# djeedai/bevy_hanabi

Hardware: AMD Instinct MI355X
Metric: particle-updates/sec (higher is better)
Workload: dtype f32

## Files before the change

### bevy_hanabi_amd/csrc/hanabi_amd.hip

```cpp
#include <hip/hip_runtime.h>

#include <algorithm>
#include <atomic>
#include <chrono>
#include <cmath>
#include <condition_variable>
#include <cstdarg>
#include <cstdio>
#include <cstring>
#include <deque>
#include <memory>
#include <mutex>
#include <string>
#include <thread>
#include <vector>

#include "hnb_kernels.hip.h"
#include "hnb_jit.h"
#include "hnb_sort.hip.h"
#include "hnb_comm.h"
#include "hnb_plan.h"
#include "hnb_export.h"
#include "hnb_export_code.inc"
#include "hnb_export_sort_code.inc"
// ... 220 lines not shown
    const char* stream_kernel_name = "";
    hipModule_t jit_module = nullptr;
    hipFunction_t jit_init = nullptr, jit_update = nullptr, jit_init_slots = nullptr;
    bool slot_init_eligible = false;
    uint32_t slot_init_frames = 0;
    uint32_t sort_skipped_frames = 0;
    uint32_t sort_path_frames[3] = {0, 0, 0};
    bool tick_sign_seen = false;
    uint64_t serial = 0;
    bool jit_pending = false;
    std::string kernel_info, jit_log;
    enum class StepsState { NotRequested, Built, Pending, Failed };
    hipModule_t steps_module = nullptr;
    hipFunction_t steps_update = nullptr;
    StepsState steps_state = StepsState::NotRequested;
    bool steps_from_cache = false;
    std::string steps_why;
    std::vector<Ins> steps_ops;
    int steps_waves = 0;
    bool steps_cohort = false;
    std::vector<Ins> h_init, h_update;
    std::string set_sig;
    uint64_t set_sig_hash = 0;
    uint32_t set_gen = 0, set_case = kNoSetCase, set_frames = 0;
    std::vector<Ins> uniform_code;
    std::vector<HnbEffect*> effects;
    uint32_t table_cap = 0;
    uint64_t* d_inst_base = nullptr;
    DevMeta* d_meta[2] = {nullptr, nullptr};
    struct SlabBlock { char* base = nullptr; uint32_t n_slots = 0; };
    std::vector<SlabBlock> slab_blocks;
    std::vector<void*> free_slabs;
    size_t slab_stride = 0;
    bool slot_order = false;
    bool has_ribbons = false;
    SortArgs sort{};
    uint32_t* d_plane_by_attr = nullptr;
    std::vector<uint32_t> parent_attrs;
    uint32_t* d_ev_totals = nullptr;
    unsigned long long* h_ev_counts = nullptr;
    uint32_t level = 0;
    uint32_t* d_counts = nullptr;
    uint32_t* d_deaths = nullptr;
    plan::SkipFacts skip_facts;
    plan::SkipHistory skip_hist;
    plan::RibbonFacts ribbon_facts;
    plan::RibbonHistory ribbon_hist;
    plan::FramePlan plan;
    const char* d_frame_cur = nullptr;
    uint32_t ring = 0;
    size_t frame_bytes = 0;
    uint32_t parity = 0;
    uint32_t frames_run = 0;
    uint32_t merged_frames = 0;
    uint32_t unmerged_frames = 0;
    bool horizon_eligible = false;
    uint32_t hz_parity = 0;
    uint32_t hz_frames = 0;
    uint32_t* d_safe = nullptr;
    unsigned long long* h_safe = nullptr;
    uint32_t* d_fault = nullptr;
    uint32_t skipped_frames = 0;
    uint32_t sort_parity = 0;
    uint32_t suffix_frames = 0;
    uint32_t sort_rotated_frames = 0;
    bool ring_live = false;
// ... 182 lines not shown
                break;
            case HNB_OP_M_POS_CONE3D:
                if (!OK(a, 3)) BAD("operand out of range");
                break;
            case HNB_OP_M_ADD_XLATE: break;
            case HNB_OP_LDPARENT:
                if (!is_init) BAD("LDPARENT outside the init stream");
                if (d + wd > file_regs) BAD("destination out of range");
                {
                    const uint32_t id = w[1] >> 16;
                    if (id >= HNB_ATTR_COUNT || id < HNB_ATTR_POSITION) BAD("parent attribute id out of range");
                    if (wd != kAttrComponents[id]) BAD("LDPARENT must read a whole attribute");
                    bool listed = false;
                    for (uint32_t k = 0; k < h.parent_n_attrs && !listed; ++k) {
                        uint32_t pid;
                        memcpy(&pid, blob_base + h.parent_attrs_off + k * 4, 4);
                        listed = pid == id;
                    }
                    if (!listed) BAD("LDPARENT of an attribute that is not in the program's parent attribute list");
                }
                break;
            case HNB_OP_M_EMIT_EVENTS:
                if (is_init) BAD("M_EMIT_EVENTS outside the update stream");
                if (!OK(a, 1)) BAD("operand out of range");
                if (((w[1] >> 16) & 0xffu) >= h.n_event_channels) BAD("event channel out of range");
                break;
            default: BAD("unhandled opcode");
        }
#undef BAD
    }
    return HNB_OK;
}

bool layout_slab(const HnbProgramHeader& h, const HnbAttrEntry* attrs, DevProgram& d, SortArgs& so, size_t* out_bytes) {
    d.capacity = h.capacity;
    d.n_attrs = h.n_attrs;
    d.n_uregs = h.n_uregs;
    d.chunks_per_inst = (h.capacity + kChunk - 1) / kChunk;
    d.init_len = h.init_len;
    d.update_len = h.update_len;
    uint64_t off = 0;
    const uint64_t list_bytes = align_up((size_t)h.capacity * 4, 256);
    auto place = [&](uint64_t bytes) { const uint64_t at = off; off += bytes; return at; };
    const uint64_t a0 = place(list_bytes), a1 = place(list_bytes), dd = place(list_bytes);
    uint64_t plane[kMaxAttrs];
    for (uint32_t i = 0; i < h.n_attrs; ++i) plane[i] = place(align_up((size_t)h.capacity * attrs[i].ncomp * 4, 256));
    const uint64_t flag_off = place(align_up((size_t)h.capacity, 256));
    const uint64_t lmin_off = place(align_up((size_t)d.chunks_per_inst * 16, 256));
    const uint64_t bit_bytes = align_up((size_t)d.chunks_per_inst * (kChunk / 8), 256);
    const uint64_t died_off = place(bit_bytes), rmask_off = place(bit_bytes);
    const uint64_t hz_off = place(align_up(256 + (size_t)d.chunks_per_inst * 24, 256));
    uint64_t ev_off[HNB_MAX_EVENT_CHANNELS] = {};
    for (uint32_t c = 0; c < h.n_event_channels; ++c) ev_off[c] = place(list_bytes);
    uint64_t key_off[2] = {}, val_off[2] = {}, hist_off = 0, gsum_off = 0, bits_off = 0;
    const bool ribbons = (h.flags & HNB_PROG_HAS_RIBBONS) != 0;
    const uint32_t sort_chunks = (h.capacity + kSortTile - 1) / kSortTile;
    if (ribbons) {
        for (int i = 0; i < 2; ++i) key_off[i] = place(align_up((size_t)h.capacity * 8, 256));
        for (int i = 0; i < 2; ++i) val_off[i] = place(list_bytes);
        hist_off = place(align_up((size_t)256 * sort_chunks * 4, 256));
        gsum_off = place(align_up((size_t)8 * ((sort_chunks + kSortGroup - 1) / kSortGroup) * 256 * 4, 256));
        bits_off = place(256);
    }
    if (off > ((uint64_t)0xffffffffu << 8)) return false;
    d.alive_off[0] = soff_of(a0); d.alive_off[1] = soff_of(a1); d.dead_off = soff_of(dd);
    for (uint32_t i = 0; i < h.n_attrs; ++i) {
        d.attrs[i].plane_off = soff_of(plane[i]);
        d.attrs[i].ncomp = attrs[i].ncomp;
        d.attrs[i].reg = attrs[i].reg;
        d.attrs[i].upd_flags = attrs[i].update_flags;
    }
    d.alive_flag_off = soff_of(flag_off);
    d.lmin_off = soff_of(lmin_off);
    d.died_bits_off = soff_of(died_off); d.row_mask_off = soff_of(rmask_off);
    d.horizon_off = soff_of(hz_off);
    d.n_event_channels = h.n_event_channels;
    for (uint32_t c = 0; c < h.n_event_channels; ++c) d.ev_cnt_off[c] = soff_of(ev_off[c]);
    if (ribbons) {
        so.capacity = h.capacity; so.chunks_per_inst = sort_chunks;
        so.alive_off[0] = d.alive_off[0]; so.alive_off[1] = d.alive_off[1];
        for (int i = 0; i < 2; ++i) { so.key_off[i] = soff_of(key_off[i]); so.val_off[i] = soff_of(val_off[i]); }
        so.hist_off = soff_of(hist_off); so.gsum_off = soff_of(gsum_off); so.bits_off = soff_of(bits_off);
        so.rid_plane.v = so.age_plane.v = kNoPlane;
        for (uint32_t i = 0; i < h.n_attrs; ++i) {
            if (attrs[i].attr == HNB_ATTR_RIBBON_ID) so.rid_plane = d.attrs[i].plane_off;
            if (attrs[i].attr == HNB_ATTR_AGE) so.age_plane = d.attrs[i].plane_off;
        }
    }
    *out_bytes = (size_t)off;
    return true;
}

int validate_blob(const void* blob, size_t size, HnbProgramHeader* out_hdr) {
    if (!blob || size < sizeof(HnbProgramHeader)) return fail(HNB_ERR_BAD_PROGRAM, "program blob too small");
    HnbProgramHeader h;
    memcpy(&h, blob, sizeof h);
// ... 486 lines not shown
            ctx->break_proof = value != 0u;
            return HNB_OK;
        }
        case HNB_OPT_TRANSPOSE: ctx->transpose = value != 0u; return HNB_OK;
        case HNB_OPT_SCENE_MERGE: ctx->scene_merge = value != 0u; return HNB_OK;
        case HNB_OPT_SUFFIX_PROOF: ctx->suffix_proof = value != 0u; return HNB_OK;
        case HNB_OPT_RING_LISTS: ctx->ring_lists = value != 0u; return HNB_OK;
        case HNB_OPT_SLOT_INIT:
            if (value > 2u) return fail(HNB_ERR_INVALID_ARG, "unknown slot-init mode %u", value);
            ctx->slot_init = value;
            return HNB_OK;
        case HNB_OPT_STREAM_HINTS: ctx->stream_hints = value != 0u; return HNB_OK;
        case HNB_OPT_DIRECT_UPLOAD: ctx->direct_upload = value != 0u; return HNB_OK;
        case HNB_OPT_JIT_ASYNC: ctx->jit_async = value != 0u; return HNB_OK;
        case HNB_OPT_FUSE_STEPS: ctx->fuse_steps = value != 0u; return HNB_OK;
        case HNB_OPT_SET_MODULE:
            if (value > HNB_SET_MODULE_BACKGROUND) return fail(HNB_ERR_INVALID_ARG, "unknown set-module mode %u", value);
            ctx->set_mode = value;
            ctx->set_lookup = plan::SetLookupState();
            return HNB_OK;
        case HNB_OPT_OVERLAP_UPDATES: ctx->overlap_updates = value != 0u && ctx->side_stream && ctx->ev_fork && ctx->ev_join; return HNB_OK;
        default: return fail(HNB_ERR_INVALID_ARG, "unknown option %u", option);
    }
}

int hnb_ctx_synchronize(HnbContext* ctx) {
    if (!ctx) return fail(HNB_ERR_INVALID_ARG, "ctx is NULL");
    HIP_TRY(hipStreamSynchronize(ctx->stream));
    return HNB_OK;
}

int hnb_program_validate(const void* blob, size_t blob_size) { return validate_blob(blob, blob_size, nullptr); }

int hnb_program_create(HnbContext* ctx, const void* blob, size_t blob_size, HnbProgram** out_prog) {
    if (!ctx || !out_prog) return fail(HNB_ERR_INVALID_ARG, "NULL argument");
    HnbProgramHeader h;
    int rc = validate_blob(blob, blob_size, &h);
    if (rc != HNB_OK) return rc;
    HIP_TRY(hipSetDevice(ctx->device));
    const uint8_t* b = static_cast<const uint8_t*>(blob);
    HnbProgram* p = new HnbProgram();
    p->ctx = ctx;
    p->hdr = h;
    p->attrs.resize(h.n_attrs);
    memcpy(p->attrs.data(), b + h.attrs_off, h.n_attrs * sizeof(HnbAttrEntry));
    p->props.resize(h.n_props);
    if (h.n_props) memcpy(p->props.data(), b + h.props_off, h.n_props * sizeof(HnbPropEntry));

    DevProgram& d = p->dev;
    size_t slab_bytes = 0;
    p->update_streams = update_is_streamable(b, h, p->attrs.data());
    if (!layout_slab(h, p->attrs.data(), d, p->sort, &slab_bytes)) { delete p; return fail(HNB_ERR_BAD_PROGRAM, "effect slab exceeds 1 TiB (capacity %u)", h.capacity); }
    p->slot_order = ctx->list_order == HNB_LIST_ORDER_SLOT && !(h.flags & HNB_PROG_HAS_RIBBONS);
    p->has_ribbons = (h.flags & HNB_PROG_HAS_RIBBONS) != 0;
    p->slab_bytes = slab_bytes;
    p->parent_attrs.resize(h.parent_n_attrs);
    if (h.parent_n_attrs) memcpy(p->parent_attrs.data(), b + h.parent_attrs_off, (size_t)h.parent_n_attrs * 4);
    {
        uint32_t planes[HNB_ATTR_COUNT];
        for (uint32_t i = 0; i < HNB_ATTR_COUNT; ++i) planes[i] = kNoPlane;
        for (uint32_t i = 0; i < h.n_attrs; ++i) planes[p->attrs[i].attr] = d.attrs[i].plane_off.v;
        hipError_t pe = hipMalloc(&p->d_plane_by_attr, sizeof planes);
        if (pe != hipSuccess) { delete p; return fail(HNB_ERR_OUT_OF_MEMORY, "hipMalloc failed: %s", hipGetErrorString(pe)); }
        hipMemcpy(p->d_plane_by_attr, planes, sizeof planes, hipMemcpyHostToDevice);
    }
    p->uniform_code.resize(h.uniform_len);
    if (h.uniform_len) memcpy(p->uniform_code.data(), b + h.uniform_off, (size_t)h.uniform_len * 8);
    p->wide_file = std::max(h.init_regs, h.update_regs) > HNB_VM_MAX_REGS;
    p->slot_init_eligible = slot_init_eligible(b, h);
    if (cull_eligible(b, h, p->attrs.data(), p->update_streams, ctx->popt, &p->cull_dt_operand)) {
        d.cull_lifetime = 1u;
        d.age_cohort = age_cohort_eligible(b, h, p->attrs.data(), p->update_streams, ctx->popt) ? 1u : 0u;
    }
    p->age_cohort_mode = ctx->popt.age_cohort;
    p->auto_materialise = ctx->popt.age_cohort == HNB_AGE_COHORT_AUTO && d.age_cohort != 0u && (h.render_reads_lo >> HNB_ATTR_AGE & 1u) != 0u;
    if (p->update_streams) select_stream_kernel(reinterpret_cast<const Ins*>(b + h.update_off), h.update_len, &p->stream_launch, &p->stream_kernel_name, &p->stream_launch_fused);
    if (!p->wide_file && jit::enabled()) {
        p->h_init.assign(reinterpret_cast<const Ins*>(b + h.init_off), reinterpret_cast<const Ins*>(b + h.init_off) + h.init_len);
        p->h_update.assign(reinterpret_cast<const Ins*>(b + h.update_off), reinterpret_cast<const Ins*>(b + h.update_off) + h.update_len);
        p->set_sig = jit::set_signature(make_set_request(p->h_init.data(), h.init_len, p->h_update.data(), h.update_len, p->attrs.data(), h.n_attrs, p->update_streams, d.age_cohort != 0u));
        p->set_sig_hash = jit::fnv1a(p->set_sig);
    }
    const bool aot_static = p->update_streams && strcmp(p->stream_kernel_name, "ProgInterp") != 0;
    p->kernel_info = std::string(p->wide_file ? "wide-file " : "") + "init=" + (h.init_len ? "interp" : "none") + " update=" +
                     (p->update_streams ? (aot_static ? std::string("aot-stream:") + p->stream_kernel_name : std::string("interp-stream")) : std::string("interp-generic"));
    p->serial = ctx->next_program_serial++;
    if (jit::enabled()) {
        const jit::Request rq = make_jit_request(b, h, p->attrs.data(), p->update_streams, aot_static, ctx->popt);
        if (rq.want_update_stream) {
            p->steps_ops.assign(rq.update, rq.update + rq.update_len);
            p->steps_waves = rq.stream_waves; p->steps_cohort = rq.stream_cohort;
        }
        jit::Result res;
        if (jit::build(rq, res, ctx->jit_async)) {
            install_program_jit(p, res);
        } else if (ctx->jit_async && res.log.empty() && (rq.want_init || rq.want_update_generic || rq.want_update_stream)) {
            std::unique_ptr<JitJob> job(new JitJob());
            job->program_serial = p->serial;
            job->blob.assign(b, b + blob_size);
            job->hdr = h; job->attrs = p->attrs; job->streams = p->update_streams; job->aot_static = aot_static; job->opt = ctx->popt;
            queue_jit_job(ctx, std::move(job));
            p->jit_pending = true;
        } else if (!res.log.empty()) {
            p->jit_log = res.log;
        }
    }
    if (p->has_ribbons && p->update_streams) {
// ... 81 lines not shown
        hipFree(p->d_plane_by_attr); hipFree(p->d_fault); hipHostFree(p->h_safe);
        delete p;
        return fail(HNB_ERR_OUT_OF_MEMORY, "hipMalloc(code) failed: %s", hipGetErrorString(e));
    }
    if (h.init_len) hipMemcpy(p->d_code, b + h.init_off, (size_t)h.init_len * 8, hipMemcpyHostToDevice);
    if (h.update_len) hipMemcpy(p->d_code + h.init_len, b + h.update_off, (size_t)h.update_len * 8, hipMemcpyHostToDevice);
    d.init_code = p->d_code;
    d.update_code = p->d_code + h.init_len;
    ctx->programs.push_back(p);
    *out_prog = p;
    return HNB_OK;
}

int hnb_program_destroy(HnbProgram* p) {
    if (!p) return HNB_OK;
    HnbContext* ctx = p->ctx;
    hipSetDevice(ctx->device);
    hipStreamSynchronize(ctx->stream);
    while (!p->effects.empty()) hnb_effect_destroy(p->effects.back());
    free_tables(p);
    if (p->jit_module) hipModuleUnload(p->jit_module);
    if (p->steps_module) hipModuleUnload(p->steps_module);
    for (auto& blk : p->slab_blocks) hipFree(blk.base);
    hipFree(p->d_plane_by_attr);
    hipFree(p->d_code);
    hipFree(p->d_fault);
    hipFree(p->d_export);
    if (p->h_safe) hipHostFree(p->h_safe);
    ctx->programs.erase(std::remove(ctx->programs.begin(), ctx->programs.end(), p), ctx->programs.end());
    delete p;
    return HNB_OK;
}

constexpr size_t kPlacementMinBytes = (size_t)256 << 20;
constexpr size_t kPlacementMaxTransient = (size_t)32 << 30;
hipError_t alloc_slab_block(HnbProgram* p, size_t bytes, char** out) {
    int want = 24;
    if (const char* e = getenv("HNB_SLAB_CANDIDATES")) want = std::max(1, std::min(32, atoi(e)));
    want = (int)std::min<size_t>((size_t)want, std::max<size_t>(1, kPlacementMaxTransient / std::max<size_t>(bytes, 1)));
    if (bytes < kPlacementMinBytes || bytes != p->slab_stride) want = 1;
    const bool debug = getenv("HNB_DEBUG_ALLOC") != nullptr;
    if (want == 1) return hipMalloc(reinterpret_cast<void**>(out), bytes);
    ProbeArgs pa{};
    pa.n_quads = (p->dev.capacity + 3u) / 4u;
    for (uint32_t a = 0; a < p->dev.n_attrs && pa.n_planes < 8; ++a) {
        const DevAttr& at = p->dev.attrs[a];
        if (at.reg == HNB_REG_NONE) continue;
        pa.off[pa.n_planes] = at.plane_off;
        pa.stride16[pa.n_planes] = at.ncomp;
        if (at.reg != HNB_REG_LIFETIME) pa.write_mask |= 1u << pa.n_planes;
        pa.n_planes += 1;
    }
    hipStream_t st = p->ctx->stream;
    hipEvent_t ev0 = nullptr, ev1 = nullptr;
    if (hipEventCreate(&ev0) != hipSuccess || hipEventCreate(&ev1) != hipSuccess) {
        if (ev0) hipEventDestroy(ev0);
        (void)hipGetLastError();
        return hipMalloc(reinterpret_cast<void**>(out), bytes);
    }
    char* best = nullptr;
    float best_ms = 0.0f;
    std::vector<float> times;
    std::vector<char*> rejected;
    hipError_t first_error = hipSuccess;
    for (int c = 0; c < want; ++c) {
        char* cand = nullptr;
        const hipError_t e = hipMalloc(reinterpret_cast<void**>(&cand), bytes);
        if (e != hipSuccess) { if (!best) first_error = e; (void)hipGetLastError(); break; }
        hipMemsetAsync(cand, 0, bytes, st);
        float ms = 1e30f;
        const uint32_t grid = (uint32_t)((pa.n_quads + 255u) / 256u);
        for (int rep = 0; rep < 4; ++rep) {
            hipEventRecord(ev0, st);
            k_probe_placement<<<grid, 256, 0, st>>>(cand, pa);
            hipEventRecord(ev1, st);
            hipEventSynchronize(ev1);
            float t = 0.0f;
            hipEventElapsedTime(&t, ev0, ev1);
            if (rep > 0 && t < ms) ms = t;
        }
        if (debug) fprintf(stderr, "hanabi_amd: slab candidate %d at %p: %.4f ms\n", c, (void*)cand, ms);
        if (!best || ms < best_ms) { if (best) rejected.push_back(best); best = cand; best_ms = ms; }
        else rejected.push_back(cand);
        times.push_back(ms);
        if (times.size() >= 3) {
            std::vector<float> sorted = times;
            std::sort(sorted.begin(), sorted.end());
            if (best_ms < 0.97f * sorted[sorted.size() / 2]) break;
        }
    }
    for (char* r : rejected) hipFree(r);
    hipEventDestroy(ev0);
    hipEventDestroy(ev1);
    if (!best) return first_error;
    *out = best;
    return hipSuccess;
}

int hnb_effect_create(HnbProgram* p, uint32_t slot_base, HnbEffect** out_fx) {
    if (!p || !out_fx) return fail(HNB_ERR_INVALID_ARG, "NULL argument");
    HnbContext* ctx = p->ctx;
    HIP_TRY(hipSetDevice(ctx->device));
    const uint32_t index = (uint32_t)p->effects.size();
    int rc = ensure_tables(p, index + 1);
    if (rc != HNB_OK) return rc;
    HIP_TRY(hipStreamSynchronize(ctx->stream));
    HnbEffect* fx = new HnbEffect();
    fx->prog = p;
    fx->index = index;
    fx->slot_base = slot_base;
    hipError_t e = hipSuccess;
    if (p->free_slabs.empty()) {
        p->slab_stride = align_up(p->slab_bytes, 64 * 1024);
        const size_t want = std::max<size_t>(1, ((size_t)1 << 30) / p->slab_stride);
        const uint32_t n_slots = (uint32_t)std::min<size_t>(want, std::max<size_t>(1, p->effects.size()));
        HnbProgram::SlabBlock blk;
        blk.n_slots = n_slots;
        e = alloc_slab_block(p, p->slab_stride * n_slots, &blk.base);
        if (e == hipSuccess) {
            p->slab_blocks.push_back(blk);
            for (uint32_t i = n_slots; i-- > 0;) p->free_slabs.push_back(blk.base + (size_t)i * p->slab_stride);
        }
    }
    if (e == hipSuccess) { fx->slab = p->free_slabs.back(); p->free_slabs.pop_back(); }
    if (e == hipSuccess && getenv("HNB_DEBUG_ALLOC")) fprintf(stderr, "hanabi_amd: effect slab %p (%zu bytes)\n", fx->slab, p->slab_bytes);
    if (e != hipSuccess) { delete fx; return fail(HNB_ERR_OUT_OF_MEMORY, "hipMalloc(%zu bytes) for effect slab failed: %s", p->slab_bytes, hipGetErrorString(e)); }
    char* base = static_cast<char*>(fx->slab);
    const uint32_t cap = p->dev.capacity;
// ... 1601 lines not shown
    if (!fx) return fail(HNB_ERR_INVALID_ARG, "fx is NULL");
    if (!fx->prog->has_ribbons) return fail(HNB_ERR_INVALID_ARG, "the particle layout has no RIBBON_ID attribute: nothing to sort");
    return HNB_OK;
}

int hnb_program_kernel_info(HnbProgram* prog, char* buf, size_t buf_size) {
    if (!prog || !buf || !buf_size) return fail(HNB_ERR_INVALID_ARG, "NULL argument");
    std::string s = prog->kernel_info;
    if (prog->jit_pending) s += " (specialisation pending: HNB_OPT_JIT_ASYNC)";
    if (!prog->jit_log.empty()) s += "\njit log: " + prog->jit_log;
    {
        const char* never = steps_never_reason(prog);
        s += "\nsteps kernel: ";
        switch (prog->steps_state) {
        case HnbProgram::StepsState::NotRequested: s += std::string("not requested") + (never ? std::string(" (") + never + ")" : std::string()); break;
        case HnbProgram::StepsState::Built: s += std::string("built") + (prog->steps_from_cache ? " (jit cache hit)" : ""); break;
        case HnbProgram::StepsState::Pending: s += "pending (HNB_OPT_JIT_ASYNC)"; break;
        case HnbProgram::StepsState::Failed: s += "failed: " + prog->steps_why; break;
        }
    }
    if (!prog->dev.age_cohort && prog->dev.cull_lifetime && prog->age_cohort_mode == HNB_AGE_COHORT_AUTO && (prog->hdr.render_reads_lo >> HNB_ATTR_AGE & 1u))
        s += "\nage cohorts: off (HNB_AGE_COHORT_AUTO: the asset's render modifiers read AGE after every frame)";
    if (prog->dev.age_cohort) {
        hipStreamSynchronize(prog->ctx->stream);
        std::vector<uint32_t> st(prog->dev.chunks_per_inst);
        size_t in_cohort = 0;
        for (const HnbEffect* fx : prog->effects) {
            if (hipMemcpy(st.data(), static_cast<const char*>(fx->slab) + prog->dev.lmin_off + (size_t)prog->dev.chunks_per_inst * 8, st.size() * 4, hipMemcpyDeviceToHost) != hipSuccess) break;
            for (uint32_t v : st) in_cohort += v == 1u ? 1u : 0u;
        }
        s += "\nage cohorts: " + std::to_string(in_cohort) + " of " + std::to_string(prog->effects.size() * (size_t)prog->dev.chunks_per_inst) + " chunks";
        if (prog->auto_materialise) s += " (HNB_AGE_COHORT_AUTO: the asset's render modifiers read AGE, the update keeps the plane current)";
    }
    if (prog->slot_init_frames) s += "\nslot-major init (large spawns): " + std::to_string(prog->slot_init_frames) + " frames";
    if (prog->has_ribbons && prog->suffix_frames) s += "\ncasualties proven to be the list's last rows (no k_count_rows): " + std::to_string(prog->suffix_frames) + " frames";
    if (prog->has_ribbons && prog->ring_frames) s += "\nlist kept as a ring (no row rewritten): " + std::to_string(prog->ring_frames) + " frames";
    if (prog->has_ribbons && prog->sort_skipped_frames) s += "\nribbon sorts skipped in list-free frames: " + std::to_string(prog->sort_skipped_frames) + " frames";
    if (prog->has_ribbons) s += "\nribbon sorts by rotation: " + std::to_string(prog->sort_rotated_frames) + " of " + std::to_string(prog->frames_run) + " frames" + (prog->ribbon_facts.front_static ? "" : " (not eligible)");
    if (prog->has_ribbons) s += "\nribbon sorts by path: one-tile " + std::to_string(prog->sort_path_frames[0]) + ", one-workgroup " + std::to_string(prog->sort_path_frames[1]) +
                                ", multi-launch " + std::to_string(prog->sort_path_frames[2]) + " frames";
    if (prog->merged_frames) s += "\nupdate served by a merged launch (small programs of the context share one): " + std::to_string(prog->merged_frames) + " frames";
    if (prog->unmerged_frames) s += "\nkept out of the shared launches (the loaded set module does not know this program; its own specialised kernels): " + std::to_string(prog->unmerged_frames) + " frames";
    if (prog->set_frames) s += "\n... by the context's set module (the program's specialised code behind the shared launch): " + std::to_string(prog->set_frames) + " frames";
    if (!prog->ctx->set_log.empty() && !prog->set_sig.empty()) s += "\nset module: " + prog->ctx->set_log;
    if (prog->ctx->set_failed_builds && !prog->set_sig.empty()) s += "\nset module builds that failed: " + std::to_string(prog->ctx->set_failed_builds);
    if (prog->horizon_eligible) s += "\ndeath horizons in use: " + std::to_string(prog->hz_frames) + " frames";
    s += "\nlists skipped: " + std::to_string(prog->skipped_frames) + " of " + std::to_string(prog->frames_run) + " frames" + (prog->skip_facts.eligible ? "" : " (not eligible)");
    s += "\nframe parameters (context): written by the host into device memory in " + std::to_string(prog->ctx->direct_frames) + " frames, copied in " + std::to_string(prog->ctx->copied_frames) +
         (prog->ctx->large_bar ? "" : " (the device memory is not host-visible: no large BAR)") + (prog->ctx->direct_failed ? " (host-visible slots failed their check)" : "");
    s += "\nhnb_simulate waited for the device (the frame " + std::to_string(kFrameRing) + " before still running) in " + std::to_string(prog->ctx->ring_waits) + " of " + std::to_string(prog->ctx->frame) +
         " frames, " + std::to_string(prog->ctx->ring_wait_ns / 1000) + " us in all";
    snprintf(buf, buf_size, "%s", s.c_str());
    return HNB_OK;
}

int hnb_jit_precompile(const void* blob, size_t blob_size) {
    HnbProgramHeader h;
    int rc = validate_blob(blob, blob_size, &h);
    if (rc != HNB_OK) return rc;
    const uint8_t* b = static_cast<const uint8_t*>(blob);
    std::vector<HnbAttrEntry> attrs(h.n_attrs);
    memcpy(attrs.data(), b + h.attrs_off, h.n_attrs * sizeof(HnbAttrEntry));
    const bool streams = update_is_streamable(b, h, attrs.data());
    bool aot_static = false;
    if (streams) {
        StreamLaunchFn fn = nullptr;
// ... 271 lines not shown
```

### bevy_hanabi_amd/csrc/hnb_kernels.hip.h

```cpp
#pragma once
#ifndef __HIPCC_RTC__
#include <hip/hip_runtime.h>
#endif
#include "hnb_dev.h"

namespace hnb {

template <class T>
__device__ __forceinline__ T* global_ptr(uint64_t addr) {
    typedef __attribute__((address_space(1))) T global_t;
    return (T*)(global_t*)addr;
}

struct u2_t { uint32_t x, y; };
struct u3_t { uint32_t x, y, z; };
typedef uint32_t u4v __attribute__((ext_vector_type(4)));
#if defined(HNB_NONTEMPORAL) || defined(HNB_NONTEMPORAL_LOADS)
#define HNB_NT_LOAD(p) __builtin_nontemporal_load(p)
#else
#define HNB_NT_LOAD(p) (*(p))
#endif
#if defined(HNB_NONTEMPORAL) || defined(HNB_NONTEMPORAL_STORES)
#define HNB_NT_STORE(v, p) __builtin_nontemporal_store(v, p)
#else
// ... 15 lines not shown
    HNB_WAVE_STEP_(v, ident, OP, 0x142, 0xa)                \
    HNB_WAVE_STEP_(v, ident, OP, 0x143, 0xc)
__device__ __forceinline__ uint32_t wave_sum_u32(uint32_t v) {
#define HNB_OP_(a, b) ((a) + (b))
    HNB_WAVE_REDUCE_(v, 0u, HNB_OP_)
#undef HNB_OP_
    return (uint32_t)__builtin_amdgcn_readlane((int)v, 63);
}
__device__ __forceinline__ uint32_t wave_min_u32(uint32_t v) {
#define HNB_OP_(a, b) ((b) < (a) ? (b) : (a))
    HNB_WAVE_REDUCE_(v, 0xffffffffu, HNB_OP_)
#undef HNB_OP_
    return (uint32_t)__builtin_amdgcn_readlane((int)v, 63);
}
__device__ __forceinline__ uint32_t wave_max_u32(uint32_t v) {
#define HNB_OP_(a, b) ((b) > (a) ? (b) : (a))
    HNB_WAVE_REDUCE_(v, 0u, HNB_OP_)
#undef HNB_OP_
    return (uint32_t)__builtin_amdgcn_readlane((int)v, 63);
}
__device__ __forceinline__ float wave_min_f32(float x) {
    uint32_t v = f2u(x);
#define HNB_OP_(a, b) f2u(fminf(u2f(a), u2f(b)))
    HNB_WAVE_REDUCE_(v, 0x7f800000u, HNB_OP_)
#undef HNB_OP_
    return u2f((uint32_t)__builtin_amdgcn_readlane((int)v, 63));
}


#ifndef HNB_JIT_TU
__global__ void k_reset_lists(uint32_t* __restrict__ dead, uint32_t* __restrict__ alive0, uint32_t* __restrict__ alive1, uint32_t capacity) {
    uint32_t i = blockIdx.x * blockDim.x + threadIdx.x;
    if (i < capacity) { dead[i] = i; alive0[i] = 0u; alive1[i] = 0u; }
}
#endif

#ifndef HNB_JIT_TU
struct ProbeArgs { uint32_t n_planes; uint32_t stride16[8]; uint64_t off[8]; uint32_t write_mask; uint32_t salt; uint64_t n_quads; };
__global__ void __launch_bounds__(256) k_probe_placement(char* __restrict__ base, const ProbeArgs a) {
    const uint64_t q = (uint64_t)blockIdx.x * 256u + threadIdx.x;
    if (q >= a.n_quads) return;
    uint32_t acc = 0;
#pragma unroll
    for (uint32_t pl = 0; pl < 8; ++pl) {
        if (pl >= a.n_planes) break;
        uint4* ptr = reinterpret_cast<uint4*>(base + a.off[pl]) + q * a.stride16[pl];
        for (uint32_t i = 0; i < a.stride16[pl]; ++i) {
            uint4 v = ptr[i];
            acc += v.x + v.y + v.z + v.w;
            v.x ^= a.salt;
            if (a.write_mask >> pl & 1u) ptr[i] = v;
        }
    }
    if (acc == 0x9e3779b9u && a.salt) *reinterpret_cast<uint32_t*>(base) = acc;
}
#endif

template <class FILE_T>
__device__ __forceinline__ void vfile_store_attr(const FILE_T& r, uint32_t ncomp, uint32_t reg, char* plane, uint32_t slot) {
    switch (ncomp) {
        case 1: reinterpret_cast<uint32_t*>(plane)[slot] = r[reg]; break;
        case 2: reinterpret_cast<u2_t*>(plane)[slot] = u2_t{r[reg], r[reg + 1]}; break;
        case 3: reinterpret_cast<u3_t*>(plane)[slot] = u3_t{r[reg], r[reg + 1], r[reg + 2]}; break;
        default: reinterpret_cast<uint4*>(plane)[slot] = make_uint4(r[reg], r[reg + 1], r[reg + 2], r[reg + 3]); break;
    }
}
__device__ __forceinline__ Out4 vfile_load_attr(uint32_t ncomp, const char* plane, uint32_t slot) {
    Out4 o = Out4{0u, 0u, 0u, 0u};
    switch (ncomp) {
        case 1: o.v0 = reinterpret_cast<const uint32_t*>(plane)[slot]; break;
        case 2: { const u2_t t = reinterpret_cast<const u2_t*>(plane)[slot]; o.v0 = t.x; o.v1 = t.y; } break;
        case 3: { const u3_t t = reinterpret_cast<const u3_t*>(plane)[slot]; o.v0 = t.x; o.v1 = t.y; o.v2 = t.z; } break;
        default: { const uint4 t = reinterpret_cast<const uint4*>(plane)[slot]; o.v0 = t.x; o.v1 = t.y; o.v2 = t.z; o.v3 = t.w; } break;
    }
    return o;
}

__device__ __forceinline__ void pin_scalar(uint32_t v) { asm volatile("" ::"s"(v)); }
__device__ __forceinline__ uint32_t requested_spawn(const DevFrameInst& f) {
    const uint4 h0 = reinterpret_cast<const uint4*>(&f)[0], h1 = reinterpret_cast<const uint4*>(&f)[1];
    const uint32_t spawn_count = h0.x, parity = h1.z, skip = h1.w;
    const uint64_t ev_in = (uint64_t)h1.x | ((uint64_t)h1.y << 32);
    pin_scalar(spawn_count);
    if (skip) return 0u;
    if (ev_in == 0ull) return spawn_count;
    const DevEventBuffer* ev = global_ptr<const DevEventBuffer>(ev_in);
    const uint2 cnt = *reinterpret_cast<const uint2*>(ev->count);
// ... 1284 lines not shown
            if (next != ast_raw) astate[j] = next;
        }
        uint32_t d = 0;
#pragma unroll
        for (uint32_t w = 0; w < kBlock / 64; ++w) d += s_died[w];
        if (d) atomicAdd(&cb.deaths[(size_t)cb.parity * cb.table_cap + k], d);
        if (d && args.skip_lists) *args.fault = 1u;
        if (args.safe_words) {
            float r = fminf(fminf(s_rem[0], s_rem[1]), fminf(s_rem[2], s_rem[3]));
            r = r > 0.0f ? r : 0.0f;
            uint32_t* word = args.safe_words + (size_t)args.safe_parity * args.safe_stride + chunk;
            if (split) atomicMin(word, f2u(r));
            else *word = f2u(r);
        }
        if (chunk_full) { if (d) cfull[j] = 0u; }
        else if (!split && d == 0u && s_alive[0] + s_alive[1] + s_alive[2] + s_alive[3] == kChunk) cfull[j] = 1u;
        if (cull && !split) {
            float m = __builtin_inff();
            bool all = true;
#pragma unroll
            for (uint32_t w = 0; w < kBlock / 64; ++w) { all = all && !(s_lmin[w] < 0.0f); m = fminf(m, s_lmin[w]); }
            if (all) lmin[j] = m < 3.0e38f ? m : 3.0e38f;
        }
    }
}

template <class PROG, int WAVES, int PROBE = 0, bool COHORT = false, bool FUSED = false>
__global__ void __launch_bounds__(kBlock, WAVES)
k_update_slots_stream(const SlotArgs args, const uint64_t* __restrict__ inst_base, const DevFrameInst* __restrict__ fi,
                      const uint32_t* __restrict__ ublocks, const CompactBufs cb) {
    update_stream_chunk<PROG, PROBE, COHORT, FUSED>(args, inst_base, fi, ublocks, cb, blockIdx.x, gridDim.x);
}
#ifndef HNB_JIT_TU
#ifndef HNB_AGEK_CUT
#define HNB_AGEK_CUT 0
#endif
__global__ void __launch_bounds__(kBlock)
k_update_slots_stream_age(const SlotArgs args, const uint64_t* __restrict__ inst_base, const DevFrameInst* __restrict__ fi,
                          const uint32_t* __restrict__ ublocks, const CompactBufs cb) {
    __shared__ uint32_t s_died[kBlock / 64], s_alive[kBlock / 64];
    __shared__ float s_lmin[kBlock / 64], s_rem[kBlock / 64];
    constexpr uint32_t kSteps = kWaveRows / kStepRows;
    const uint32_t tid = threadIdx.x, lane = tid & 63u, wave = tid >> 6;
    const uint32_t wg = blockIdx.x, wg_total = gridDim.x;
    const uint32_t chunk = chunk_of_workgroup(cb.xcd_remap, wg, wg_total);
    const uint32_t k = chunk / args.chunks_per_inst, j = chunk - k * args.chunks_per_inst;
    const uint32_t frozen = fi[k].skip;
    char* base = global_ptr<char>(inst_base[k]);
    const float dt_tick = u2f(ublocks[(size_t)k * args.n_uregs + (args.dt_operand & 0xffu)]);
    char* p_age = base + args.plane_off[2];
    const char* p_life = base + args.plane_off[3];
    uint32_t* flags4 = reinterpret_cast<uint32_t*>(base + args.alive_flag_off);
    float* lmin = reinterpret_cast<float*>(base + args.lmin_off);
    uint32_t* cfull = reinterpret_cast<uint32_t*>(lmin) + args.chunks_per_inst;
    const uint32_t wave0 = j * kChunk + wave * kWaveRows;
    uint32_t f4s[kSteps];
    u4v ages[kSteps];
#pragma unroll
    for (uint32_t step = 0; step < kSteps; ++step) {
        const uint32_t s0 = wave0 + step * kStepRows + lane * 4u;
        const bool in = s0 < args.capacity;
        f4s[step] = in ? ld_hint(flags4 + (s0 >> 2), args.stream_hint != 0u) : 0u;
        ages[step] = in ? reinterpret_cast<const u4v*>(p_age)[s0 >> 2] : u4v{0u, 0u, 0u, 0u};
    }
    const uint32_t cf = cfull[j];
    const float Lm = lmin[j];
// ... 420 lines not shown
```

### bevy_hanabi_amd/csrc/hnb_plan.h

```cpp
#pragma once
#include <cstdint>
#include <cstring>

namespace hnb {
namespace plan {

struct InstanceFrame {
    bool simulated = true;
    bool has_parent = false;
    uint32_t spawn_count = 0;
    uint32_t event_capacity = 0;
    const uint32_t* ublock = nullptr;
};
inline uint32_t uword(const InstanceFrame& f, uint32_t decoded_operand) { return f.ublock[decoded_operand & 0xffu]; }
inline float as_float(uint32_t bits) { float f; std::memcpy(&f, &bits, 4); return f; }
inline bool nonneg_not_nan(uint32_t float_bits) { return float_bits <= 0x7f800000u; }

struct SkipFacts {
    bool eligible = false;
    uint32_t dt_operand = 0;
};
struct SkipHistory {
    double cum_tick[128] = {};
    uint32_t last_dirty = 0;
// ... 225 lines not shown

inline void partition_init_passes(const uint8_t* reads, uint32_t n, int heavy, uint8_t* side) {
    for (uint32_t i = 0; i < n; ++i) side[i] = heavy >= 0 ? 1u : 0u;
    if (heavy < 0) return;
    side[heavy] = 0u;
    for (uint32_t c = 0; c < n; ++c)
        if (reads[c * n + (uint32_t)heavy]) side[c] = 0u;
    for (bool changed = true; changed;) {
        changed = false;
        for (uint32_t c = 0; c < n; ++c)
            if (!side[c])
                for (uint32_t p = 0; p < n; ++p)
                    if (side[p] && reads[c * n + p]) { side[p] = 0u; changed = true; }
    }
}

struct SetLookupState { uint64_t seen = 0, tried = 0; };
inline bool set_lookup_due(SetLookupState& st, bool enabled, bool job_running, bool covered, uint32_t n_candidates, uint64_t population) {
    if (!enabled || job_running || covered || n_candidates < 2u) return false;
    if (population == st.tried) return false;
    if (population != st.seen) { st.seen = population; return false; }
    st.tried = population;
    return true;
}

constexpr uint64_t kStreamHintBytes = 256ull << 20;
inline bool use_streaming_hints(uint64_t total_slots, uint32_t update_bytes_per_slot) {
    return total_slots * (uint64_t)(update_bytes_per_slot + 8u) > kStreamHintBytes;
}

constexpr uint64_t kStoreHintBytes = 384ull << 20;
inline bool use_store_hints(uint64_t total_slots, uint32_t stored_bytes_per_slot) { return total_slots * (uint64_t)stored_bytes_per_slot > kStoreHintBytes; }

struct FramePlan {
    bool skip_lists = false;
    bool lists = true;
    bool lists_merged = false;
    bool hz_use = false;
    bool stream_hint = false;
    bool store_hint = false;
    RibbonDecision ribbon;
    bool independent = false;
    MergeDecision merge;
    uint32_t init_blocks = 0;
    SlotInitDecision slot_init;
};

}
}
```

Measured before the change: 123.1 billion.

## Make slab placement probe mimic the streaming update kernel and refine candidate selection

Reworks the physical-placement search for large effect slabs. The probe kernel now mirrors the streaming update's chunk/wave access pattern, XCD remap, occupancy and per-plane load/store masks, so candidate timings better reflect the real update. The stop rule now distinguishes a single timing class from multiple classes and keeps searching for a while after the best candidate. It also adds optional per-plane skew padding (off by default), a per-program stream-wave choice, and diagnostics. The cost is more allocation-time probing, and the probe may still mispredict real performance.

```diff
diff --git a/bevy_hanabi_amd/csrc/hanabi_amd.hip b/bevy_hanabi_amd/csrc/hanabi_amd.hip
--- a/bevy_hanabi_amd/csrc/hanabi_amd.hip
+++ b/bevy_hanabi_amd/csrc/hanabi_amd.hip
@@ -276,6 +276,10 @@
     std::vector<SlabBlock> slab_blocks;
     std::vector<void*> free_slabs;
     size_t slab_stride = 0;
+    uint32_t plane_pad[kMaxAttrs] = {};
+    int stream_waves = HNB_STREAM_WAVES;
+    uint32_t placement_tried = 0;
+    float placement_best_ms = 0.0f, placement_median_ms = 0.0f;
     bool slot_order = false;
     bool has_ribbons = false;
     SortArgs sort{};
@@ -524,36 +528,27 @@
     return HNB_OK;
 }
 
-bool layout_slab(const HnbProgramHeader& h, const HnbAttrEntry* attrs, DevProgram& d, SortArgs& so, size_t* out_bytes) {
+bool layout_slab(const HnbProgramHeader& h, const HnbAttrEntry* attrs, DevProgram& d, SortArgs& so, size_t* out_bytes, const uint32_t* pad256 = nullptr) {
     d.capacity = h.capacity;
     d.n_attrs = h.n_attrs;
     d.n_uregs = h.n_uregs;
     d.chunks_per_inst = (h.capacity + kChunk - 1) / kChunk;
     d.init_len = h.init_len;
     d.update_len = h.update_len;
-    uint64_t off = 0;
-    const uint64_t list_bytes = align_up((size_t)h.capacity * 4, 256);
-    auto place = [&](uint64_t bytes) { const uint64_t at = off; off += bytes; return at; };
-    const uint64_t a0 = place(list_bytes), a1 = place(list_bytes), dd = place(list_bytes);
-    uint64_t plane[kMaxAttrs];
-    for (uint32_t i = 0; i < h.n_attrs; ++i) plane[i] = place(align_up((size_t)h.capacity * attrs[i].ncomp * 4, 256));
-    const uint64_t flag_off = place(align_up((size_t)h.capacity, 256));
-    const uint64_t lmin_off = place(align_up((size_t)d.chunks_per_inst * 16, 256));
-    const uint64_t bit_bytes = align_up((size_t)d.chunks_per_inst * (kChunk / 8), 256);
-    const uint64_t died_off = place(bit_bytes), rmask_off = place(bit_bytes);
-    const uint64_t hz_off = place(align_up(256 + (size_t)d.chunks_per_inst * 24, 256));
-    uint64_t ev_off[HNB_MAX_EVENT_CHANNELS] = {};
-    for (uint32_t c = 0; c < h.n_event_channels; ++c) ev_off[c] = place(list_bytes);
-    uint64_t key_off[2] = {}, val_off[2] = {}, hist_off = 0, gsum_off = 0, bits_off = 0;
-    const bool ribbons = (h.flags & HNB_PROG_HAS_RIBBONS) != 0;
+    static_assert(plan::kLayoutMaxAttrs == kMaxAttrs && plan::kLayoutMaxChannels == HNB_MAX_EVENT_CHANNELS, "plan::SlabShape limits");
+    plan::SlabShape shape;
+    shape.capacity = h.capacity; shape.n_attrs = h.n_attrs; shape.n_event_channels = h.n_event_channels;
+    shape.ribbons = (h.flags & HNB_PROG_HAS_RIBBONS) != 0;
+    shape.chunk = kChunk; shape.sort_tile = kSortTile; shape.sort_group = kSortGroup;
+    for (uint32_t i = 0; i < h.n_attrs; ++i) { shape.ncomp[i] = attrs[i].ncomp; shape.pad256[i] = pad256 ? pad256[i] : 0u; }
+    const plan::SlabSections sec = plan::layout_sections(shape);
+    const uint64_t off = sec.total, a0 = sec.alive[0], a1 = sec.alive[1], dd = sec.dead;
+    const uint64_t* plane = sec.plane;
+    const uint64_t flag_off = sec.flag, lmin_off = sec.lmin, died_off = sec.died, rmask_off = sec.rmask, hz_off = sec.horizon;
+    const uint64_t* ev_off = sec.ev;
+    const uint64_t *key_off = sec.key, *val_off = sec.val, hist_off = sec.hist, gsum_off = sec.gsum, bits_off = sec.bits;
+    const bool ribbons = shape.ribbons;
     const uint32_t sort_chunks = (h.capacity + kSortTile - 1) / kSortTile;
-    if (ribbons) {
-        for (int i = 0; i < 2; ++i) key_off[i] = place(align_up((size_t)h.capacity * 8, 256));
-        for (int i = 0; i < 2; ++i) val_off[i] = place(list_bytes);
-        hist_off = place(align_up((size_t)256 * sort_chunks * 4, 256));
-        gsum_off = place(align_up((size_t)8 * ((sort_chunks + kSortGroup - 1) / kSortGroup) * 256 * 4, 256));
-        bits_off = place(256);
-    }
     if (off > ((uint64_t)0xffffffffu << 8)) return false;
     d.alive_off[0] = soff_of(a0); d.alive_off[1] = soff_of(a1); d.dead_off = soff_of(dd);
     for (uint32_t i = 0; i < h.n_attrs; ++i) {
@@ -1106,6 +1101,13 @@
 
 int hnb_program_validate(const void* blob, size_t blob_size) { return validate_blob(blob, blob_size, nullptr); }
 
+constexpr size_t kPlacementMinBytes = (size_t)256 << 20;
+constexpr uint32_t kPlaneSkewBytes = 0;
+uint32_t plane_skew_for(size_t slab_bytes) {
+    if (const char* e = getenv("HNB_PLANE_SKEW")) return (uint32_t)(std::min<long long>(std::max(0ll, atoll(e)), 1ll << 30) / 256);
+    return slab_bytes >= kPlacementMinBytes ? kPlaneSkewBytes / 256u : 0u;
+}
+
 int hnb_program_create(HnbContext* ctx, const void* blob, size_t blob_size, HnbProgram** out_prog) {
     if (!ctx || !out_prog) return fail(HNB_ERR_INVALID_ARG, "NULL argument");
     HnbProgramHeader h;
@@ -1125,6 +1127,10 @@
     size_t slab_bytes = 0;
     p->update_streams = update_is_streamable(b, h, p->attrs.data());
     if (!layout_slab(h, p->attrs.data(), d, p->sort, &slab_bytes)) { delete p; return fail(HNB_ERR_BAD_PROGRAM, "effect slab exceeds 1 TiB (capacity %u)", h.capacity); }
+    if (const uint32_t skew256 = plane_skew_for(slab_bytes)) {
+        for (uint32_t i = 1; i < h.n_attrs; ++i) p->plane_pad[i] = skew256;
+        if (!layout_slab(h, p->attrs.data(), d, p->sort, &slab_bytes, p->plane_pad)) { delete p; return fail(HNB_ERR_BAD_PROGRAM, "effect slab exceeds 1 TiB (capacity %u)", h.capacity); }
+    }
     p->slot_order = ctx->list_order == HNB_LIST_ORDER_SLOT && !(h.flags & HNB_PROG_HAS_RIBBONS);
     p->has_ribbons = (h.flags & HNB_PROG_HAS_RIBBONS) != 0;
     p->slab_bytes = slab_bytes;
@@ -1147,6 +1153,12 @@
         d.age_cohort = age_cohort_eligible(b, h, p->attrs.data(), p->update_streams, ctx->popt) ? 1u : 0u;
     }
     p->age_cohort_mode = ctx->popt.age_cohort;
+    {
+        bool lean = true;
+        for (uint32_t i = 0; i < h.update_len; ++i) lean = lean && vm_op_is_lean(reinterpret_cast<const Ins*>(b + h.update_off)[i].x & 0xffu);
+        p->stream_waves = lean ? HNB_STREAM_WAVES : HNB_STREAM_WAVES_FULL;
+        if (d.age_cohort && p->stream_waves > HNB_STREAM_WAVES_COHORT) p->stream_waves = HNB_STREAM_WAVES_COHORT;
+    }
     p->auto_materialise = ctx->popt.age_cohort == HNB_AGE_COHORT_AUTO && d.age_cohort != 0u && (h.render_reads_lo >> HNB_ATTR_AGE & 1u) != 0u;
     if (p->update_streams) select_stream_kernel(reinterpret_cast<const Ins*>(b + h.update_off), h.update_len, &p->stream_launch, &p->stream_kernel_name, &p->stream_launch_fused);
     if (!p->wide_file && jit::enabled()) {
@@ -1294,25 +1306,54 @@
     return HNB_OK;
 }
 
-constexpr size_t kPlacementMinBytes = (size_t)256 << 20;
 constexpr size_t kPlacementMaxTransient = (size_t)32 << 30;
+constexpr int kPlacementCandidates = 24;
+size_t placement_min_bytes() {
+    if (const char* e = getenv("HNB_SLAB_MIN_BYTES")) return (size_t)std::max(0ll, atoll(e));
+    return kPlacementMinBytes;
+}
+ProbeArgs probe_args_of(const HnbProgram* p) {
+    ProbeArgs pa{};
+    pa.stream = p->update_streams ? 1u : 0u;
+    pa.n_quads = ((uint64_t)p->dev.capacity + 3u) / 4u;
+    for (uint32_t a = 0; a < p->dev.n_attrs && pa.n_planes < 4; ++a) {
+        const DevAttr& at = p->dev.attrs[a];
+        if (at.reg == HNB_REG_NONE || at.ncomp > 3u) continue;
+        bool load = (at.upd_flags & HNB_ATTR_UPD_LOAD) != 0, store = (at.upd_flags & HNB_ATTR_UPD_STORE) != 0;
+        if (pa.stream) {
+            if (at.reg == HNB_REG_LIFETIME && p->dev.cull_lifetime) load = false;
+            if (at.reg == HNB_REG_AGE && p->dev.age_cohort) { load = false; store = store && p->auto_materialise; }
+        } else {
+            load = true; store = store || at.reg != HNB_REG_LIFETIME;
+        }
+        if (!load && !store) continue;
+        const uint32_t i = pa.n_planes++;
+        pa.off[i] = at.plane_off;
+        pa.ncomp[i] = at.ncomp;
+        pa.words[i] = align_up((size_t)p->dev.capacity * at.ncomp * 4, 256) / 16;
+        if (load) pa.load_mask |= 1u << i;
+        if (store) pa.store_mask |= 1u << i;
+    }
+    return pa;
+}
+void launch_probe(int waves, uint32_t grid, hipStream_t st, char* block, const ProbeArgs& pa) {
+    const size_t lds = pa.stream ? sizeof(StreamLds) : 0;
+    switch (waves) {
+    case 4: k_probe_placement<4><<<grid, kBlock, lds, st>>>(block, pa); break;
+    case 5: k_probe_placement<5><<<grid, kBlock, lds, st>>>(block, pa); break;
+    default: k_probe_placement<6><<<grid, kBlock, lds, st>>>(block, pa); break;
+    }
+}
 hipError_t alloc_slab_block(HnbProgram* p, size_t bytes, char** out) {
-    int want = 24;
+    int want = kPlacementCandidates;
     if (const char* e = getenv("HNB_SLAB_CANDIDATES")) want = std::max(1, std::min(32, atoi(e)));
     want = (int)std::min<size_t>((size_t)want, std::max<size_t>(1, kPlacementMaxTransient / std::max<size_t>(bytes, 1)));
-    if (bytes < kPlacementMinBytes || bytes != p->slab_stride) want = 1;
+    if (bytes < placement_min_bytes() || bytes != p->slab_stride) want = 1;
     const bool debug = getenv("HNB_DEBUG_ALLOC") != nullptr;
     if (want == 1) return hipMalloc(reinterpret_cast<void**>(out), bytes);
-    ProbeArgs pa{};
-    pa.n_quads = (p->dev.capacity + 3u) / 4u;
-    for (uint32_t a = 0; a < p->dev.n_attrs && pa.n_planes < 8; ++a) {
-        const DevAttr& at = p->dev.attrs[a];
-        if (at.reg == HNB_REG_NONE) continue;
-        pa.off[pa.n_planes] = at.plane_off;
-        pa.stride16[pa.n_planes] = at.ncomp;
-        if (at.reg != HNB_REG_LIFETIME) pa.write_mask |= 1u << pa.n_planes;
-        pa.n_planes += 1;
-    }
+    ProbeArgs pa = probe_args_of(p);
+    if (pa.n_planes == 0u) return hipMalloc(reinterpret_cast<void**>(out), bytes);
+    const uint32_t grid = pa.stream ? p->dev.chunks_per_inst : (uint32_t)((pa.n_quads + kBlock - 1u) / kBlock);
     hipStream_t st = p->ctx->stream;
     hipEvent_t ev0 = nullptr, ev1 = nullptr;
     if (hipEventCreate(&ev0) != hipSuccess || hipEventCreate(&ev1) != hipSuccess) {
@@ -1320,42 +1361,41 @@
         (void)hipGetLastError();
         return hipMalloc(reinterpret_cast<void**>(out), bytes);
     }
-    char* best = nullptr;
-    float best_ms = 0.0f;
     std::vector<float> times;
-    std::vector<char*> rejected;
+    std::vector<char*> cands;
     hipError_t first_error = hipSuccess;
+    plan::PlacementPick pick;
     for (int c = 0; c < want; ++c) {
         char* cand = nullptr;
         const hipError_t e = hipMalloc(reinterpret_cast<void**>(&cand), bytes);
-        if (e != hipSuccess) { if (!best) first_error = e; (void)hipGetLastError(); break; }
+        if (e != hipSuccess) { if (cands.empty()) first_error = e; (void)hipGetLastError(); break; }
         hipMemsetAsync(cand, 0, bytes, st);
         float ms = 1e30f;
-        const uint32_t grid = (uint32_t)((pa.n_quads + 255u) / 256u);
-        for (int rep = 0; rep < 4; ++rep) {
+        for (int rep = 0; rep < 5; ++rep) {
+            pa.mode = (p->ctx->alternate && (rep & 1)) ? 2u : 0u;
             hipEventRecord(ev0, st);
-            k_probe_placement<<<grid, 256, 0, st>>>(cand, pa);
+            launch_probe(p->stream_waves, grid, st, cand, pa);
             hipEventRecord(ev1, st);
-            hipEventSynchronize(ev1);
             float t = 0.0f;
-            hipEventElapsedTime(&t, ev0, ev1);
+            if (hipEventSynchronize(ev1) != hipSuccess || hipEventElapsedTime(&t, ev0, ev1) != hipSuccess) { (void)hipGetLastError(); continue; }
             if (rep > 0 && t < ms) ms = t;
         }
         if (debug) fprintf(stderr, "hanabi_amd: slab candidate %d at %p: %.4f ms\n", c, (void*)cand, ms);
-        if (!best || ms < best_ms) { if (best) rejected.push_back(best); best = cand; best_ms = ms; }
-        else rejected.push_back(cand);
+        cands.push_back(cand);
         times.push_back(ms);
-        if (times.size() >= 3) {
-            std::vector<float> sorted = times;
-            std::sort(sorted.begin(), sorted.end());
-            if (best_ms < 0.97f * sorted[sorted.size() / 2]) break;
-        }
-    }
-    for (char* r : rejected) hipFree(r);
+        pick = plan::placement_pick(times.data(), (uint32_t)times.size(), (uint32_t)want);
+        if (pick.stop) break;
+    }
     hipEventDestroy(ev0);
     hipEventDestroy(ev1);
-    if (!best) return first_error;
-    *out = best;
+    if (cands.empty()) return first_error;
+    pick = plan::placement_pick(times.data(), (uint32_t)times.size(), (uint32_t)times.size());
+    for (size_t i = 0; i < cands.size(); ++i) if (i != pick.pick) hipFree(cands[i]);
+    std::vector<float> sorted = times;
+    std::sort(sorted.begin(), sorted.end());
+    p->placement_tried = (uint32_t)times.size(); p->placement_best_ms = times[pick.pick]; p->placement_median_ms = sorted[sorted.size() / 2];
+    if (debug) fprintf(stderr, "hanabi_amd: slab placement: %u candidates, kept %u (%.4f ms, median %.4f ms)\n", p->placement_tried, pick.pick, p->placement_best_ms, p->placement_median_ms);
+    *out = cands[pick.pick];
     return hipSuccess;
 }
 
@@ -3023,6 +3063,15 @@
         s += "\nage cohorts: " + std::to_string(in_cohort) + " of " + std::to_string(prog->effects.size() * (size_t)prog->dev.chunks_per_inst) + " chunks";
         if (prog->auto_materialise) s += " (HNB_AGE_COHORT_AUTO: the asset's render modifiers read AGE, the update keeps the plane current)";
     }
+    {
+        char line[256];
+        if (prog->placement_tried) snprintf(line, sizeof line, "\nslab placement: %u candidates tried, best %.4f ms, median %.4f ms", prog->placement_tried, prog->placement_best_ms, prog->placement_median_ms);
+        else snprintf(line, sizeof line, "\nslab placement: not searched");
+        s += line;
+        s += "; plane skews (bytes):";
+        uint64_t cum = 0;
+        for (uint32_t i = 0; i < prog->dev.n_attrs; ++i) { cum += (uint64_t)prog->plane_pad[i] * 256u; s += " " + std::to_string(cum); }
+    }
     if (prog->slot_init_frames) s += "\nslot-major init (large spawns): " + std::to_string(prog->slot_init_frames) + " frames";
     if (prog->has_ribbons && prog->suffix_frames) s += "\ncasualties proven to be the list's last rows (no k_count_rows): " + std::to_string(prog->suffix_frames) + " frames";
     if (prog->has_ribbons && prog->ring_frames) s += "\nlist kept as a ring (no row rewritten): " + std::to_string(prog->ring_frames) + " frames";
diff --git a/bevy_hanabi_amd/csrc/hnb_kernels.hip.h b/bevy_hanabi_amd/csrc/hnb_kernels.hip.h
--- a/bevy_hanabi_amd/csrc/hnb_kernels.hip.h
+++ b/bevy_hanabi_amd/csrc/hnb_kernels.hip.h
@@ -71,27 +71,6 @@
 __global__ void k_reset_lists(uint32_t* __restrict__ dead, uint32_t* __restrict__ alive0, uint32_t* __restrict__ alive1, uint32_t capacity) {
     uint32_t i = blockIdx.x * blockDim.x + threadIdx.x;
     if (i < capacity) { dead[i] = i; alive0[i] = 0u; alive1[i] = 0u; }
-}
-#endif
-
-#ifndef HNB_JIT_TU
-struct ProbeArgs { uint32_t n_planes; uint32_t stride16[8]; uint64_t off[8]; uint32_t write_mask; uint32_t salt; uint64_t n_quads; };
-__global__ void __launch_bounds__(256) k_probe_placement(char* __restrict__ base, const ProbeArgs a) {
-    const uint64_t q = (uint64_t)blockIdx.x * 256u + threadIdx.x;
-    if (q >= a.n_quads) return;
-    uint32_t acc = 0;
-#pragma unroll
-    for (uint32_t pl = 0; pl < 8; ++pl) {
-        if (pl >= a.n_planes) break;
-        uint4* ptr = reinterpret_cast<uint4*>(base + a.off[pl]) + q * a.stride16[pl];
-        for (uint32_t i = 0; i < a.stride16[pl]; ++i) {
-            uint4 v = ptr[i];
-            acc += v.x + v.y + v.z + v.w;
-            v.x ^= a.salt;
-            if (a.write_mask >> pl & 1u) ptr[i] = v;
-        }
-    }
-    if (acc == 0x9e3779b9u && a.salt) *reinterpret_cast<uint32_t*>(base) = acc;
 }
 #endif
 
@@ -1442,6 +1421,81 @@
     update_stream_chunk<PROG, PROBE, COHORT, FUSED>(args, inst_base, fi, ublocks, cb, blockIdx.x, gridDim.x);
 }
 #ifndef HNB_JIT_TU
+struct ProbeArgs {
+    uint32_t n_planes;
+    uint32_t ncomp[4];
+    uint64_t off[4];
+    uint64_t words[4];
+    uint32_t load_mask, store_mask;
+    uint32_t salt;
+    uint32_t stream;
+    uint32_t mode;
+    uint64_t n_quads;
+};
+template <int WAVES>
+__global__ void __launch_bounds__(kBlock) __attribute__((amdgpu_waves_per_eu(WAVES, WAVES))) k_probe_placement(char* __restrict__ base, const ProbeArgs a) {
+    uint32_t acc = 0;
+    if (!a.stream) {
+        const uint64_t q = (uint64_t)blockIdx.x * kBlock + threadIdx.x;
+        if (q >= a.n_quads) return;
+#pragma unroll
+        for (uint32_t pl = 0; pl < 4; ++pl) {
+            if (pl >= a.n_planes || !((a.load_mask | a.store_mask) >> pl & 1u)) continue;
+            u4v* ptr = reinterpret_cast<u4v*>(base + a.off[pl]);
+            for (uint32_t i = 0; i < a.ncomp[pl]; ++i) {
+                const uint64_t g = q * a.ncomp[pl] + i;
+                if (g >= a.words[pl]) break;
+                u4v v = u4v{0u, 0u, 0u, 0u};
+                if (a.load_mask >> pl & 1u) { v = ptr[g]; acc += v.x + v.y + v.z + v.w; v.x ^= a.salt; }
+                if (a.store_mask >> pl & 1u) ptr[g] = v;
+            }
+        }
+    } else {
+        const uint32_t lane = threadIdx.x & 63u, wave = threadIdx.x >> 6;
+        const uint32_t chunk = chunk_of_workgroup(a.mode, blockIdx.x, gridDim.x);
+        constexpr uint32_t kSteps = kWaveRows / kStepRows;
+        auto word_of = [&](uint32_t pl, uint32_t step, uint32_t w) {
+            return ((uint64_t)chunk * (kChunk / 4u) + wave * (kWaveRows / 4u)) * a.ncomp[pl] + (step * a.ncomp[pl] + w) * 64u + lane;
+        };
+#pragma unroll
+        for (uint32_t pl = 0; pl < 4; ++pl) {
+            if (pl >= a.n_planes || !(a.store_mask >> pl & 1u) || (a.load_mask >> pl & 1u)) continue;
+            u4v* ptr = reinterpret_cast<u4v*>(base + a.off[pl]);
+            for (uint32_t step = 0; step < kSteps; ++step)
+                for (uint32_t w = 0; w < a.ncomp[pl]; ++w) { const uint64_t g = word_of(pl, step, w); if (g < a.words[pl]) ptr[g] = u4v{a.salt, 0u, 0u, 0u}; }
+        }
+        constexpr int kInFlight = WAVES <= 4 ? 2 : 1;
+#pragma unroll kInFlight
+        for (uint32_t step = 0; step < kSteps; ++step) {
+            u4v v[4][3];
+#pragma unroll
+            for (uint32_t pl = 0; pl < 4; ++pl) {
+                if (pl >= a.n_planes || !(a.load_mask >> pl & 1u)) continue;
+                const u4v* ptr = reinterpret_cast<const u4v*>(base + a.off[pl]);
+#pragma unroll
+                for (uint32_t w = 0; w < 3; ++w) {
+                    v[pl][w] = u4v{0u, 0u, 0u, 0u};
+                    if (w < a.ncomp[pl]) { const uint64_t g = word_of(pl, step, w); if (g < a.words[pl]) v[pl][w] = ptr[g]; }
+                }
+            }
+#pragma unroll
+            for (uint32_t pl = 0; pl < 4; ++pl) {
+                if (pl >= a.n_planes || !(a.load_mask >> pl & 1u)) continue;
+                u4v* ptr = reinterpret_cast<u4v*>(base + a.off[pl]);
+#pragma unroll
+                for (uint32_t w = 0; w < 3; ++w) {
+                    if (w >= a.ncomp[pl]) continue;
+                    acc += v[pl][w].x + v[pl][w].y + v[pl][w].z + v[pl][w].w;
+                    v[pl][w].x ^= a.salt;
+                    const uint64_t g = word_of(pl, step, w);
+                    if ((a.store_mask >> pl & 1u) && g < a.words[pl]) ptr[g] = v[pl][w];
+                }
+            }
+        }
+    }
+    if (acc == 0x9e3779b9u && a.salt) *reinterpret_cast<uint32_t*>(base + a.off[0]) = acc;
+}
+
 #ifndef HNB_AGEK_CUT
 #define HNB_AGEK_CUT 0
 #endif
diff --git a/bevy_hanabi_amd/csrc/hnb_plan.h b/bevy_hanabi_amd/csrc/hnb_plan.h
--- a/bevy_hanabi_amd/csrc/hnb_plan.h
+++ b/bevy_hanabi_amd/csrc/hnb_plan.h
@@ -281,6 +281,72 @@
 constexpr uint64_t kStoreHintBytes = 384ull << 20;
 inline bool use_store_hints(uint64_t total_slots, uint32_t stored_bytes_per_slot) { return total_slots * (uint64_t)stored_bytes_per_slot > kStoreHintBytes; }
 
+constexpr uint32_t kLayoutMaxAttrs = 40, kLayoutMaxChannels = 8;
+struct SlabShape {
+    uint32_t capacity = 0, n_attrs = 0;
+    uint32_t ncomp[kLayoutMaxAttrs] = {};
+    uint32_t pad256[kLayoutMaxAttrs] = {};
+    uint32_t n_event_channels = 0;
+    bool ribbons = false;
+    uint32_t chunk = 4096, sort_tile = 4096, sort_group = 32;
+};
+struct SlabSections {
+    uint64_t alive[2] = {}, dead = 0, plane[kLayoutMaxAttrs] = {}, flag = 0, lmin = 0, died = 0, rmask = 0, horizon = 0, ev[kLayoutMaxChannels] = {};
+    uint64_t key[2] = {}, val[2] = {}, hist = 0, gsum = 0, bits = 0;
+    uint64_t total = 0;
+};
+inline uint64_t up256(uint64_t v) { return (v + 255u) & ~(uint64_t)255u; }
+inline SlabSections layout_sections(const SlabShape& s) {
+    SlabSections o;
+    uint64_t off = 0;
+    auto place = [&](uint64_t bytes) { const uint64_t at = off; off += bytes; return at; };
+    const uint64_t list_bytes = up256((uint64_t)s.capacity * 4u);
+    const uint64_t chunks = ((uint64_t)s.capacity + s.chunk - 1u) / s.chunk;
+    o.alive[0] = place(list_bytes); o.alive[1] = place(list_bytes); o.dead = place(list_bytes);
+    for (uint32_t i = 0; i < s.n_attrs && i < kLayoutMaxAttrs; ++i) { off += (uint64_t)s.pad256[i] * 256u; o.plane[i] = place(up256((uint64_t)s.capacity * s.ncomp[i] * 4u)); }
+    o.flag = place(up256(s.capacity));
+    o.lmin = place(up256(chunks * 16u));
+    const uint64_t bit_bytes = up256(chunks * (s.chunk / 8u));
+    o.died = place(bit_bytes); o.rmask = place(bit_bytes);
+    o.horizon = place(up256(256u + chunks * 24u));
+    for (uint32_t c = 0; c < s.n_event_channels && c < kLayoutMaxChannels; ++c) o.ev[c] = place(list_bytes);
+    if (s.ribbons) {
+        const uint64_t sort_chunks = ((uint64_t)s.capacity + s.sort_tile - 1u) / s.sort_tile;
+        for (int i = 0; i < 2; ++i) o.key[i] = place(up256((uint64_t)s.capacity * 8u));
+        for (int i = 0; i < 2; ++i) o.val[i] = place(list_bytes);
+        o.hist = place(up256(256u * sort_chunks * 4u));
+        o.gsum = place(up256(8u * ((sort_chunks + s.sort_group - 1u) / s.sort_group) * 256u * 4u));
+        o.bits = place(256u);
+    }
+    o.total = off;
+    return o;
+}
+
+constexpr float kPlacementSeparation = 0.97f;
+constexpr uint32_t kPlacementStand = 12, kPlacementOneClass = 8;
+constexpr float kPlacementFailed = 1e29f;
+struct PlacementPick { bool stop = true; uint32_t pick = 0; };
+inline PlacementPick placement_pick(const float* ms, uint32_t n, uint32_t budget) {
+    PlacementPick r;
+    if (n == 0u) { r.stop = budget == 0u; return r; }
+    bool have = false;
+    float best = 0.0f, worst = 0.0f;
+    uint32_t finite = 0;
+    for (uint32_t i = 0; i < n; ++i) {
+        if (!(ms[i] < kPlacementFailed)) continue;
+        finite += 1u;
+        if (!have || ms[i] < best) { best = ms[i]; r.pick = i; }
+        if (!have || ms[i] > worst) worst = ms[i];
+        have = true;
+    }
+    if (n >= budget) { r.stop = true; return r; }
+    if (!have) { r.stop = false; return r; }
+    const bool classes = best < kPlacementSeparation * worst;
+    if (!classes) { r.stop = finite >= kPlacementOneClass; return r; }
+    r.stop = n - 1u - r.pick >= kPlacementStand;
+    return r;
+}
+
 struct FramePlan {
     bool skip_lists = false;
     bool lists = true;
```

Result: slower. 118.8 billion (-3.5%).
